# CityU-AIM-Group/HTD

Measured on AMD Instinct MI355X. Metric: images/sec (1333x800) HTD-R50 train step, higher is better.
Workload: dtype f32; 1 GPU; HTD ResNet-50 FPN fp32 train step fwd+bwd+SGD, batch 4/GPU @ 1333x800 (padded 1344x800), random-init weights, 2000 RPN proposals/img, 512 RoIs/img/stage; global_batch=4, parallelism=dp1, stage2_positives=158, proposals=random-init RPN (few positives: the regression branch is nearly idle)

## Files before the change

### htd_amd/csrc/conv_x3.hip

```cpp
#include <algorithm>
#include <mutex>
#include <type_traits>
#include <unordered_map>

#include <stdlib.h>

#include "common.h"

namespace {

using f32x16 = __attribute__((ext_vector_type(16))) float;
using bf16x8 = __attribute__((ext_vector_type(8))) __bf16;
using bf16x2 = __attribute__((ext_vector_type(2))) __bf16;
using f32x2 = __attribute__((ext_vector_type(2))) float;
using f32x4 = __attribute__((ext_vector_type(4))) float;

using f16x8 = __attribute__((ext_vector_type(8))) _Float16;
using f16x2 = __attribute__((ext_vector_type(2))) _Float16;

constexpr int XK = 16;
constexpr int NCH = 6;

struct H2Scale { float s, inv; };
__device__ __forceinline__ H2Scale h2_scale(const float *amax)
// ... 302 lines not shown
                *reinterpret_cast<float4 *>(p.y + o) = v;
                omax = absmax4(omax, v);
                if (p.yp != nullptr) emit_planes4(p.yp, p.yp_rows, m, n, v);
            } else {
                auto put = [&](int e, float t) {
                    if (n + e >= p.Co) return;
                    t += p.bias ? p.bias[n + e] : 0.f;
                    if (p.residual) t += p.residual[o + e];
                    if (p.relu) t = fmaxf(t, 0.f);
                    if (p.mask_src) t = p.mask_src[o + e] > 0.f ? t : 0.f;
                    p.y[o + e] = t;
                    omax = absmax4(omax, make_float4(t, 0.f, 0.f, 0.f));
                };
                put(0, v.x); put(1, v.y); put(2, v.z); put(3, v.w);
            }
        }
        if (i + 1 < TM) __syncthreads();
    }
    if (p.amax_out != nullptr && !part) block_absmax_out(omax, p.amax_out, le, oseen);
}

template <int WGM, int WGN, int TM, int TN, int KW, int NB, bool H2 = false>
constexpr int x3p_occupancy()
{
    constexpr int BM = WGM * TM * 32, BN = WGN * TN * 32;
    constexpr int NCHL = H2 ? 4 : NCH;
    constexpr int main_bytes = (2 * NCHL * Geo<BM, KW>::PITCH + NB * NCHL * BN) * 16;
    constexpr int epi_bytes = WGM * 32 * (BN + 4) * 4;
    constexpr int by_lds = 163840 / (main_bytes > epi_bytes ? main_bytes : epi_bytes);
    constexpr int by_regs = TM * TN >= 4 ? (H2 && HTD_X3H_OCC4 ? 4 : 3) : 4;
    return by_lds < by_regs ? by_lds : by_regs;
}

template <int WGM, int WGN, int TM, int TN, int KW, bool MF16, int NB, bool H2 = false>
__global__ __launch_bounds__(256, (x3p_occupancy<WGM, WGN, TM, TN, KW, NB, H2>())) void conv_x3p_kernel(X3Params p)
{
    static_assert(!(H2 && MF16), "H2: 32x32x16 form only");
    constexpr int NCHL = H2 ? 4 : NCH;
    constexpr int BM = WGM * TM * 32, BN = WGN * TN * 32;
    using G = Geo<BM, KW>;
    constexpr int PADX = (KW - 1) / 2;
    constexpr int A_VEC = NCHL * G::PITCH;
    constexpr int B_VEC = NCHL * BN;
    constexpr int MAIN_VEC = 2 * A_VEC + NB * B_VEC;
    constexpr int EPI_STRIDE = BN + 4, EPI_ROWS = WGM * 32;
    constexpr int EPI_VEC = EPI_ROWS * EPI_STRIDE / 4;
    constexpr int LDS_VEC = MAIN_VEC > EPI_VEC ? MAIN_VEC : EPI_VEC;
    __shared__ uint4 lds[LDS_VEC];
    uint4 *const lA = lds, *const lB = lds + 2 * A_VEC;
    const unsigned lds_a0 = (unsigned)(size_t)(__attribute__((address_space(3))) void *)lA;

    int bid = blockIdx.x, split = 0, sps = 0;
    bool part = false;
    const bool region_b = bid >= p.tiles_a * p.splits_a;
    if (region_b) {
        const int r = bid - p.tiles_a * p.splits_a;
        bid = p.tiles_a + r / p.splits_b;
        split = r % p.splits_b;
        part = p.splits_b > 1;
        sps = p.sps_b;
    } else if (p.splits_a > 1) {
        split = bid % p.splits_a;
        bid = bid / p.splits_a;
        part = true;
        sps = p.sps_a;
    } else {
        const int q = p.tiles_a / 8, r = p.tiles_a % 8, xcd = bid % 8, idx = bid / 8;
        bid = (xcd < r ? xcd * (q + 1) : r * (q + 1) + (xcd - r) * q) + idx;
    }
    const int tile_m = bid / p.nt, tile_n = bid % p.nt;
    const int64_t m0 = (int64_t)tile_m * BM;
    const int n0 = tile_n * BN;

    const int tid = threadIdx.x, lane = tid & 63, wave = tid >> 6;
    const int wm = wave / WGN, wn = wave % WGN;
    const int frow = lane & 31, fhalf = lane >> 5;
    const int PADY = (p.kh - 1) / 2;

    const int vcol = tid & 3, vrow = tid >> 2;
    const int a_g0 = (int)m0 + vrow - PADX;
    unsigned a_off[KW > 1 ? 1 : G::PASSES];
    bool a_in[KW > 1 ? 1 : G::PASSES];
    unsigned a_tm[KW > 1 ? 1 : G::PASSES];
    if constexpr (KW > 1) {
        a_off[0] = (unsigned)a_g0 * (unsigned)p.Ci + vcol * 4;
// ... 346 lines not shown
                    for (int i = 0; i < NP; ++i) store_pass(abuf ^ 1, i, (P ^ 1) * NP + i);
                } else {
                    store_pass(abuf ^ 1, kx, P ^ 1);
                }
            }
        }
        lds_barrier();
        bbuf = bbuf + 1 == NB ? 0 : bbuf + 1;
        if (++kx == KW) {
            kx = 0;
            ++s;
            abuf ^= 1;
            cs = cs1; ky = ky1;
            cs1 = cs2; ky1 = ky2;
            if (++ky2 == p.kh) { ky2 = 0; ++cs2; }
            n1shift = n2shift; n1koff = n2koff;
            n2shift = (ky2 - PADY) * p.Wx;
            n2koff = tap_koff(ky2, cs2);
        }
    };
    const int taps_total = (s_end - s_begin) * KW;
    int t = 0;
#pragma unroll 1
    for (; t + 1 < taps_total; t += 2) {
        tap(0, false);
        tap(1, false);
    }
    if (t < taps_total) tap(0, true);
    wait_vm<0>();
#pragma unroll
    for (int i = 0; i < 2 * NPT; ++i) landed(ra[i]);

    x3_epilogue<WGM, WGN, TM, TN, MF16>(p, acc, lds, m0, n0, part, region_b, split);
}

template <int WGM, int WGN, int TM, int TN, int NS>
constexpr int x3q_occupancy()
{
    constexpr int BM = WGM * TM * 32, BN = WGN * TN * 32;
    constexpr int main_bytes = NS * NCH * (BM + BN) * 16;
    constexpr int epi_bytes = WGM * 32 * (BN + 4) * 4;
    constexpr int by_lds = 163840 / (main_bytes > epi_bytes ? main_bytes : epi_bytes);
    constexpr int by_regs = TM * TN >= 4 ? 3 : 4;
    return by_lds < by_regs ? by_lds : by_regs;
}

template <int WGM, int WGN, int TM, int TN, bool MF16, int NS>
__global__ __launch_bounds__(256, (x3q_occupancy<WGM, WGN, TM, TN, NS>())) void conv_x3q_kernel(X3Params p)
{
    constexpr int BM = WGM * TM * 32, BN = WGN * TN * 32;
    constexpr int A_VEC = NCH * BM, B_VEC = NCH * BN;
    constexpr int MAIN_VEC = NS * (A_VEC + B_VEC);
    constexpr int EPI_VEC = WGM * 32 * (BN + 4) / 4;
    constexpr int LDS_VEC = MAIN_VEC > EPI_VEC ? MAIN_VEC : EPI_VEC;
    __shared__ uint4 lds[LDS_VEC];
    uint4 *const lA = lds, *const lB = lds + NS * A_VEC;
    const unsigned lds_a0 = (unsigned)(size_t)(__attribute__((address_space(3))) void *)lA;
    const unsigned lds_b0 = (unsigned)(size_t)(__attribute__((address_space(3))) void *)lB;

    int bid = blockIdx.x, split = 0, sps = 0;
    bool part = false;
    const bool region_b = bid >= p.tiles_a * p.splits_a;
    if (region_b) {
        const int r = bid - p.tiles_a * p.splits_a;
        bid = p.tiles_a + r / p.splits_b;
        split = r % p.splits_b;
// ... 737 lines not shown
        case 0: hipLaunchKernelGGL((conv_x3p_kernel<2, 2, 1, 1, 1, false, HTD_X3H_NB, true>), grid, dim3(256), 0, s, p); break;
        case 1: hipLaunchKernelGGL((conv_x3p_kernel<2, 2, 2, 2, 1, false, HTD_X3H_NB, true>), grid, dim3(256), 0, s, p); break;
        case 2: hipLaunchKernelGGL((conv_x3p_kernel<2, 2, 2, 1, 1, false, HTD_X3H_NB, true>), grid, dim3(256), 0, s, p); break;
        default: hipLaunchKernelGGL((conv_x3p_kernel<2, 2, 1, 2, 1, false, HTD_X3H_NB, true>), grid, dim3(256), 0, s, p); break;
        }
    } else if (p.xp != nullptr) {
        switch (cfg) {
        case 0: launch_tile_q<1, 1>(p, grid, s); break;
        case 1: launch_tile_q<2, 2>(p, grid, s); break;
        case 2: launch_tile_q<2, 1>(p, grid, s); break;
        default: launch_tile_q<1, 2>(p, grid, s); break;
        }
    } else {
        switch (cfg) {
        case 0: launch_tile<1, 1>(p, kw, grid, s); break;
        case 1: launch_tile<2, 2>(p, kw, grid, s); break;
        case 2: launch_tile<2, 1>(p, kw, grid, s); break;
        default: launch_tile<1, 2>(p, kw, grid, s); break;
        }
    }
    if (pl.partial_floats > 0) {
        const int64_t rows = (p.splits_a > 1 ? p.m_rem0 : 0) + (p.splits_b > 1 ? p.M - p.m_rem0 : 0);
        if ((p.Co & 3) == 0) {
            const unsigned rb = (unsigned)std::min<int64_t>(htd::ceil_div(rows * (p.Co >> 2), 256), p.amax_out ? 1024 : 4096);
            hipLaunchKernelGGL(conv_x3p_splitk_epilogue_vec_kernel, dim3(rb), dim3(256), 0, s, p);
        } else {
            const unsigned rb = (unsigned)std::min<int64_t>(htd::ceil_div(rows * p.Co, 256), p.amax_out ? 1024 : 4096);
            hipLaunchKernelGGL(conv_x3p_splitk_epilogue_kernel, dim3(rb), dim3(256), 0, s, p);
        }
    }
    return htd::check_launch("conv2d_x3p");
}

bool x3h_strided_ok(int Ci, int Co, int kh, int kw, int stride, int pad)
{
    static const bool on = !(getenv("HTD_X3H_STRIDED") && atoi(getenv("HTD_X3H_STRIDED")) == 0);
    return on && Ci % XK == 0 && Co >= 33 && kh == 3 && kw == 3 && stride == 2 && pad == 1;
}

bool x3p_shape_ok(int Ci, int Co, int kh, int kw, int stride, int pad, int dil)
{
    if (Ci % XK != 0 || Co < 33 || dil != 1 || kh != kw) return false;
    if (kh == 1) return pad == 0 && stride >= 1;
    return kh == 3 && stride == 1 && pad == 1;
}

}

extern "C" int htd_conv2d_x3p_supported(int Ci, int Co, int kh, int kw, int stride, int pad, int dil)
{
    return (!x3p_off() && htd::conv_math() == 1 && x3p_shape_ok(Ci, Co, kh, kw, stride, pad, dil)) ? 1 : 0;
}

int g_conv_h2 = getenv("HTD_CONV_H2") ? atoi(getenv("HTD_CONV_H2")) : 1;
extern "C" int htd_conv2d_set_h2(int on)
{
    const int prev = g_conv_h2;
    if (on == 0 || on == 1) g_conv_h2 = on;
    return prev;
}
extern "C" int htd_conv2d_x3h_supported(int Ci, int Co, int kh, int kw, int stride, int pad, int dil)
{
    return (g_conv_h2 == 1 && htd_conv2d_x3p_supported(Ci, Co, kh, kw, stride, pad, dil)) ? 1 : 0;
}
extern "C" int htd_conv2d_x3h_strided_supported(int Ci, int Co, int kh, int kw, int stride, int pad, int dil)
{
// ... 221 lines not shown
        p.res_H = res_h; p.res_W = res_w;
        p.res_sh = (float)res_h / (float)p.Ho; p.res_sw = (float)res_w / (float)p.Wo;
    }
    if (taps) {
        p.kh = p.ntl = kh * kw;
        for (int t = 0; t < p.ntl; ++t) { p.tl_dy[t] = t / kw - pad; p.tl_dx[t] = t % kw - pad; p.tl_w[t] = t; }
        return launch_x3p(p, 1, (hipStream_t)stream, workspace);
    }
    return launch_x3p(p, kw, (hipStream_t)stream, workspace);
}

extern "C" int htd_conv2d_bwd_data_x3h(const float *gy, const float *amax, const void *wplanesT, const float *mask_src,
                                       const float *accum, float *gx, void *gxplanes, float *amax_out, int B, int H, int W,
                                       int Ci, int Co, int kh, int kw, int pad, void *workspace, void *stream)
{
    HTD_REQUIRE(!gxplanes || Ci % XK == 0, "conv2d_bwd_data_x3h: output planes need Ci %% 16 == 0 (Ci=%d)", Ci);
    HTD_REQUIRE(gy && amax && wplanesT && gx && B > 0 && H > 0 && W > 0, "conv2d_bwd_data_x3h: bad arguments");
    HTD_REQUIRE(x3p_shape_ok(Co, Ci, kh, kw, 1, pad, 1), "conv2d_bwd_data_x3h: unsupported layer Ci=%d Co=%d k=%dx%d p=%d", Ci, Co, kh,
                kw, pad);
    X3Params p{};
    p.x = gy; p.wp = (const uint4 *)wplanesT; p.residual = accum; p.mask_src = mask_src; p.y = gx;
    p.Hx = H; p.Wx = W; p.Ho = H; p.Wo = W;
    p.Ci = Co; p.Co = Ci; p.Cop = planes_np(Ci); p.kh = kh; p.stride = 1;
    p.M = (int64_t)B * H * W;
    p.ncs = Co / XK;
    p.amax = amax;
    p.wscale = reinterpret_cast<const float *>(p.wp + planes_vec(kh * kw, Co, p.Cop));
    p.yp = (uint4 *)gxplanes; p.yp_rows = act_rows(p.M);
    p.amax_out = amax_out;
    HTD_REQUIRE((int64_t)B * H * W * Co < (1ll << 31), "conv2d_bwd_data_x3h: operand too large");
    return launch_x3p(p, kw, (hipStream_t)stream, workspace);
}

namespace {
struct StridedClass { int ntaps; int dy[9], dx[9], w[9]; int Ho, Wo; };
int strided_classes(int H, int W, int kh, int kw, int stride, int pad, StridedClass *cls)
{
    int n = 0;
    for (int c = 0; c < stride * stride; ++c) {
        const int ph = c / stride, pw = c % stride;
        StridedClass &q = cls[c];
        q.ntaps = 0;
        q.Ho = ph < H ? (H - ph + stride - 1) / stride : 0;
        q.Wo = pw < W ? (W - pw + stride - 1) / stride : 0;
        if (q.Ho == 0 || q.Wo == 0) continue;
        for (int ky = 0; ky < kh; ++ky) {
            const int ry = ph + pad - ky;
            if (((ry % stride) + stride) % stride != 0) continue;
            for (int kx = 0; kx < kw; ++kx) {
                const int rx = pw + pad - kx;
                if (((rx % stride) + stride) % stride != 0) continue;
                q.dy[q.ntaps] = ry >= 0 ? ry / stride : -((-ry) / stride);
                q.dx[q.ntaps] = rx >= 0 ? rx / stride : -((-rx) / stride);
                q.w[q.ntaps] = (kh - 1 - ky) * kw + (kw - 1 - kx);
                ++q.ntaps;
            }
        }
        n += q.ntaps > 0;
    }
    return n;
}
bool x3h_strided_dgrad_ok(int Ci, int Co, int kh, int kw, int stride, int pad)
{
    static const bool on = !(getenv("HTD_X3H_STRIDED") && atoi(getenv("HTD_X3H_STRIDED")) == 0);
    return on && Co % XK == 0 && Ci >= 33 && stride == 2 && ((kh == 3 && kw == 3 && pad == 1) || (kh == 1 && kw == 1 && pad == 0));
}
}

extern "C" int htd_conv2d_bwd_data_x3h_strided_supported(int Ci, int Co, int kh, int kw, int stride, int pad, int dil)
{
    return (g_conv_h2 == 1 && !x3p_off() && htd::conv_math() == 1 && dil == 1 && x3h_strided_dgrad_ok(Ci, Co, kh, kw, stride, pad)) ? 1 : 0;
}

extern "C" int64_t htd_conv2d_bwd_data_x3h_strided_workspace_bytes(int B, int H, int W, int Ci, int Co, int kh, int kw, int stride, int pad)
{
    if (!x3h_strided_dgrad_ok(Ci, Co, kh, kw, stride, pad) || B <= 0 || H <= 0 || W <= 0) return 0;
    StridedClass cls[4];
    strided_classes(H, W, kh, kw, stride, pad, cls);
    int64_t need = 0;
    for (int c = 0; c < stride * stride; ++c)
        if (cls[c].ntaps > 0)
            need = std::max(need, htd_conv2d_x3p_workspace_bytes((int64_t)B * cls[c].Ho * cls[c].Wo, Ci, Co, cls[c].ntaps, 1));
    return need;
}

extern "C" int htd_conv2d_bwd_data_x3h_strided(const float *gy, const float *amax, const void *wplanesT, const float *mask_src,
                                               float *gx, float *amax_out, int B, int H, int W, int Ci, int Co, int kh, int kw,
                                               int stride, int pad, void *workspace, void *stream)
{
    HTD_REQUIRE(gy && amax && wplanesT && gx && B > 0 && H > 0 && W > 0, "conv2d_bwd_data_x3h_strided: bad arguments");
    HTD_REQUIRE(x3h_strided_dgrad_ok(Ci, Co, kh, kw, stride, pad), "conv2d_bwd_data_x3h_strided: unsupported layer Ci=%d Co=%d k=%dx%d s=%d p=%d",
                Ci, Co, kh, kw, stride, pad);
    const int Ho = (H + 2 * pad - kh) / stride + 1, Wo = (W + 2 * pad - kw) / stride + 1;
    HTD_REQUIRE(Ho > 0 && Wo > 0 && (int64_t)B * Ho * Wo * Co < (1ll << 31) && (int64_t)B * H * W * Ci < (1ll << 40),
                "conv2d_bwd_data_x3h_strided: bad sizes");
    StridedClass cls[4];
    const int live = strided_classes(H, W, kh, kw, stride, pad, cls);
    if (live < stride * stride) {
        if (hipMemsetAsync(gx, 0, (size_t)B * H * W * Ci * 4, (hipStream_t)stream) != hipSuccess) {
            htd::set_error("conv2d_bwd_data_x3h_strided: memset failed");
            return HTD_ERR_LAUNCH;
        }
    }
    X3Params p{};
    p.x = gy; p.wp = (const uint4 *)wplanesT; p.mask_src = mask_src; p.y = gx;
    p.Hx = Ho; p.Wx = Wo;
    p.Ci = Co; p.Co = Ci; p.Cop = planes_np(Ci); p.stride = 1;
    p.ncs = Co / XK;
    p.amax = amax;
    p.wscale = reinterpret_cast<const float *>(p.wp + planes_vec(kh * kw, Co, p.Cop));
    p.amax_out = amax_out;
    p.o_step = stride; p.oH = H; p.oW = W;
    for (int c = 0; c < stride * stride; ++c) {
        const StridedClass &q = cls[c];
        if (q.ntaps == 0) continue;
        X3Params r = p;
        r.Ho = q.Ho; r.Wo = q.Wo;
        r.M = (int64_t)B * q.Ho * q.Wo;
        r.kh = r.ntl = q.ntaps;
        for (int t = 0; t < q.ntaps; ++t) { r.tl_dy[t] = q.dy[t]; r.tl_dx[t] = q.dx[t]; r.tl_w[t] = q.w[t]; }
        r.o_h0 = c / stride; r.o_w0 = c % stride;
        const int st = launch_x3p(r, 1, (hipStream_t)stream, workspace);
        if (st) return st;
    }
    return HTD_OK;
}
```

### htd_amd/dense.py

```python
import os

import torch
from torch.autograd import Function
from torch.autograd.function import once_differentiable
from torch.multiprocessing.reductions import StorageWeakRef as _StorageWeakRef

from . import capi
from .mmcv_ops import chain_outputs

CL = torch.channels_last
_P = capi.ptr
_S = capi.current_stream_ptr


def _out_hw(H, W, kh, kw, stride, pad, dil):
    return ((H + 2 * pad - (dil * (kh - 1) + 1)) // stride + 1, (W + 2 * pad - (dil * (kw - 1) + 1)) // stride + 1)


def _need_gpu(t, name):
    if not t.is_cuda:
        raise NotImplementedError(f'{name}: only GPU tensors are supported (libhtd_amd.so has no CPU path)')


def _splitk_ws(M, Co, Cred, kh, kw, device):
    nbytes = capi.lib().htd_conv2d_workspace_bytes(M, Co, Cred, kh, kw)
    return torch.empty(nbytes // 4, device=device, dtype=torch.float32) if nbytes > 0 else None


_GRAD_SINK = {}


def register_grad_sinks(params, views, used):
# ... 739 lines not shown
    else:
        capi.call('htd_conv2d_bwd_weight', _P(x), _P(g), _P(gw), _P(gb), B, H, W, Ci, Co, kh, kw, stride, padding,
                  dilation, _P(ws), _S(), work=work)
    return gw, gb, sink_w and sink_b


def _wgrad_raw(x, g, weight, stride, padding, dilation, bias=None, overlap=True):
    amax = _wgrad_amax(x, g, weight, stride, padding, dilation)
    if not overlap or not OVERLAP_WGRAD or (capi.profiling() and not _OVERLAP_IN_PROFILE):
        if OVERLAP_WGRAD and _SIDE and SINK_ACCUMULATE and grad_sink_again(weight) is not None:
            torch.cuda.current_stream().wait_stream(side_stream(g.device))
        return _wgrad_launch(x, g, weight, stride, padding, dilation, bias, amax)[:2]
    main, side = torch.cuda.current_stream(), side_stream(g.device)
    side.wait_stream(main)
    x.record_stream(side)
    g.record_stream(side)
    with torch.cuda.stream(side):
        gw, gb, sinks = _wgrad_launch(x, g, weight, stride, padding, dilation, bias, amax)
    if not sinks and not side_consumed(weight):
        if gw is not None:
            gw.record_stream(main)
        if gb is not None:
            gb.record_stream(main)
        main.wait_stream(side)
    return gw, gb


def _dgrad_joined(galias, g, weight, x_shape, stride, padding, dilation):
    fuse = galias is not None and stride == 1 and galias.dtype == g.dtype and tuple(galias.shape) == tuple(x_shape)
    gx = _dgrad_raw(g, weight, x_shape, stride, padding, dilation, accum=galias.contiguous(memory_format=CL) if fuse else None)
    return gx if (galias is None or fuse) else gx + galias


class Conv2dFunction(Function):
    @staticmethod
    def forward(ctx, x, weight, bias, residual, stride, padding, dilation, relu, res_up=False, chain=False):
        _need_gpu(x, 'conv2d')
        src = x
        x = x.contiguous(memory_format=CL)
        weight = weight.contiguous(memory_format=CL)
        res = residual.contiguous(memory_format=CL) if residual is not None else None
        b = bias.contiguous() if bias is not None else None
        y = _fwd_raw(x, weight, b, res, stride, padding, dilation, relu, res_up)
        ctx.save_for_backward(x, weight, y if relu else None)
        ctx.cfg = (stride, padding, dilation, bool(relu), bias is not None, residual is not None)
        ctx.res_up = tuple(res.shape) if (res_up and res is not None) else None
        ctx.bias_ref = b
        return chain_outputs(ctx, y, (src, ), chain)

    @staticmethod
    @once_differentiable
    def backward(ctx, g, galias=None):
        x, weight, y = ctx.saved_tensors
        stride, padding, dilation, relu, has_bias, has_res = ctx.cfg
        if g is None:
            return (galias, ) + (None, ) * 9
        g = g.contiguous(memory_format=CL)
        need_x, need_w, need_b, need_r = ctx.needs_input_grad[:4]
        gb = gw = None
        want_b = has_bias and need_b
        if relu:
            if want_b and not need_w:
                g, gb = _colsum_raw(g, y, ctx.bias_ref)
            else:
                g = _mask_raw(g, y)
        elif want_b and not need_w:
# ... 25 lines not shown
        b1 = b1.contiguous() if b1 is not None else None
        b2 = b2.contiguous() if b2 is not None else None
        h = _fwd_raw(x, w1, b1, None, 1, padding, 1, True)
        y = _fwd_raw(h, w2, b2, None, 1, 0, 1, False)
        ctx.save_for_backward(x, w1, w2, h)
        ctx.cfg = (int(padding), b1, b2)
        return chain_outputs(ctx, y, (src, ), chain)

    @staticmethod
    @once_differentiable
    def backward(ctx, gy, galias=None):
        x, w1, w2, h = ctx.saved_tensors
        padding, b1, b2 = ctx.cfg
        if gy is None:
            return (galias, ) + (None, ) * 6
        need_x, need_w1, need_b1, need_w2, need_b2 = ctx.needs_input_grad[:5]
        gy = gy.contiguous(memory_format=CL)
        gw1 = gb1 = gw2 = gb2 = None
        if need_w2:
            gw2, gb2 = _wgrad_raw(h, gy, w2, 1, 0, 1, b2 if (need_b2 and b2 is not None) else None)
        elif need_b2 and b2 is not None:
            gb2 = _colsum_raw(gy, None, b2)[1]
        gh = _dgrad_raw(gy, w2, h.shape, 1, 0, 1, mask_src=h)
        if need_w1:
            gw1, gb1 = _wgrad_raw(x, gh, w1, 1, padding, 1, b1 if (need_b1 and b1 is not None) else None)
        elif need_b1 and b1 is not None:
            gb1 = _colsum_raw(gh, None, b1)[1]
        gx = _dgrad_joined(galias, gh, w1, x.shape, 1, padding, 1) if need_x else galias
        return gx, gw1, gb1, gw2, gb2, None, None


def conv_relu_head(x, w1, b1, w2, b2, padding=1, chain=False):
    return ConvReluHeadFunction.apply(x, w1, b1, w2, b2, int(padding), bool(chain))



def _gconv_pack(weight, groups, transpose):
    C, cg, kh, kw = weight.shape
    n = capi.lib().htd_gconv2d_packed_floats(C, groups, kh, kw)
    if n <= 0:
        raise ValueError(f'grouped conv2d: {C} channels in {groups} groups is unsupported')
    wp = torch.empty(n, device=weight.device, dtype=weight.dtype)
    capi.call('htd_gconv2d_pack_weights', _P(weight), _P(wp), C, groups, kh, kw, int(transpose), _S())
    return wp


def _gconv_fwd_raw(x, wp, bias, geom, relu, cols_shape=None):
    C, groups, kh, kw, stride, padding, dilation = geom
    B, H, W = cols_shape if cols_shape is not None else (x.size(0), x.size(2), x.size(3))
    Ho, Wo = _out_hw(H, W, kh, kw, stride, padding, dilation)
    y = torch.empty((B, C, Ho, Wo), device=x.device, dtype=x.dtype, memory_format=CL)
    capi.call('htd_gconv2d_fwd', _P(x), _P(wp), _P(bias), _P(y), B, H, W, C, groups, kh, kw, stride, padding, dilation,
              int(bool(relu)), int(cols_shape is not None), _S(),
              work=('flop', 2.0 * B * Ho * Wo * C * kh * kw * (C // groups), 4.0 * (x.numel() + y.numel())))
    return y


def _gconv_dgrad_raw(g, wpT, geom, x_shape, cols=False):
    C, groups, kh, kw, stride, padding, dilation = geom
    B, _, H, W = x_shape
    M = g.size(0) * g.size(2) * g.size(3)
    gx = torch.empty((M, kh * kw, C), device=g.device, dtype=g.dtype) if cols else \
        torch.empty((B, C, H, W), device=g.device, dtype=g.dtype, memory_format=CL)
    capi.call('htd_gconv2d_bwd_data', _P(g), _P(wpT), _P(gx), B, H, W, C, groups, kh, kw, stride, padding, dilation,
              int(cols), _S(), work=('flop', 2.0 * M * C * kh * kw * (C // groups), 4.0 * (g.numel() + gx.numel())))
    return gx
# ... 565 lines not shown
```

### htd_amd/detector/rpn_head.py

```python
import torch

from ..core import multi_apply
from ..core.bbox import delta2bbox_clip_device
from ..core.misc import arange_cached, const_tensor
from .. import mmcv_ops as M
from ..mmcv_ops import nms_sorted_mask
from ..registry import HEADS
from .anchor_heads import AnchorHead
from .bricks import Conv2d, normal_init


class _RPNLossFunction(torch.autograd.Function):

    @staticmethod
    def forward(ctx, cls, reg, anchors, gts, assigned, pos, neg, means, stds, beta, pos_weight):
        from .. import capi
        from ..core.bbox import _f4
        B, A = assigned.shape
        K = gts.size(1)
        cls, reg = cls.float().contiguous(), reg.float().contiguous()
        anchors, gts = anchors.float().contiguous(), gts.float().contiguous()
        assigned = assigned.contiguous()
        pos8, neg8 = pos.to(torch.uint8).contiguous(), neg.to(torch.uint8).contiguous()
        partial = torch.empty(capi.lib().htd_rpn_loss_partial_rows(), 2, device=cls.device, dtype=torch.float32)
# ... 92 lines not shown
        super().__init__(1, in_channels, **kwargs)
        assert self.use_sigmoid_cls and not self.reg_decoded_bbox, 'HTD configs use a sigmoid RPN with delta targets'

    def _init_layers(self):
        self.rpn_conv = Conv2d(self.in_channels, self.feat_channels, 3, padding=1)
        self.rpn_cls = Conv2d(self.feat_channels, self.num_anchors * self.cls_out_channels, 1)
        self.rpn_reg = Conv2d(self.feat_channels, self.num_anchors * 4, 1)

    def init_weights(self):
        normal_init(self.rpn_conv, std=0.01)
        normal_init(self.rpn_cls, std=0.01)
        normal_init(self.rpn_reg, std=0.01)

    def forward_single(self, x):
        x = self.rpn_conv(x, relu=True)
        if x.dtype != torch.float32:
            x = x.float()
        return self.rpn_cls(x), self.rpn_reg(x)

    def forward(self, feats):
        if not feats[0].is_cuda:
            return multi_apply(self.forward_single, feats)
        nc, nr = self.rpn_cls.out_channels, self.rpn_reg.out_channels
        pad = -(nc + nr) % 8
        w = torch.cat([self.rpn_cls.weight, self.rpn_reg.weight] +
                      ([self.rpn_cls.weight.new_zeros(pad, *self.rpn_cls.weight.shape[1:])] if pad else []))
        b = torch.cat([self.rpn_cls.bias, self.rpn_reg.bias] + ([self.rpn_cls.bias.new_zeros(pad)] if pad else []))
        cls, reg, merged = [], [], []
        taps = isinstance(feats, M.PyramidTaps)
        from .. import dense
        if torch.is_grad_enabled() and w.requires_grad:
            dense.temp_grad_sink(w)
            dense.temp_grad_sink(b)
        for i in range(len(feats)):
            x = feats[i]
            if x.dtype == torch.float32 and x.size(1) % 8 == 0:
                conv = (self.rpn_conv.weight, self.rpn_conv.bias, w, b, self.rpn_conv.padding[0])
                y = feats.tap(lambda f: dense.conv_relu_head(f, *conv, True), i)[0] if taps else dense.conv_relu_head(x, *conv)
            else:
                h = self.rpn_conv(x, relu=True)
                if h.dtype != torch.float32:
                    h = h.float()
                y = self.rpn_cls(h, weight=w, bias=b)
            merged.append(y)
        if RPN_FLAT_HEADS and self.cls_out_channels == 1 and nr == 4 * nc and all(y.dtype == torch.float32 for y in merged):
            cls_all, reg_all = _RPNGatherHeads.apply(nc, *merged)
            cls, reg, off = LevelList(), LevelList(), 0
            B = cls_all.size(0)
            for y in merged:
                hh, ww = y.size(2), y.size(3)
                n = hh * ww * nc
                cls.append(cls_all[:, off:off + n].view(B, hh, ww, nc).permute(0, 3, 1, 2))
                reg.append(reg_all[:, off:off + n].reshape(B, hh, ww, nr).permute(0, 3, 1, 2))
                off += n
            cls.flat, reg.flat = cls_all, reg_all
            return cls, reg
        for y in merged:
            c, r = _SplitHeads.apply(y, nc, nr)
            cls.append(c)
            reg.append(r)
        return cls, reg

    def simple_test_rpn(self, x, img_metas):
        return self.get_bboxes(*self(x), img_metas)

    def aug_test_rpn(self, feats, img_metas):
        from ..core.post_processing import merge_aug_proposals
        samples_per_gpu = len(img_metas[0])
        aug_proposals = [[] for _ in range(samples_per_gpu)]
        for x, img_meta in zip(feats, img_metas):
# ... 201 lines not shown
```

### include/htd_amd.h

```cpp
#ifndef HTD_AMD_H
#define HTD_AMD_H

#include <stdint.h>

#ifdef __cplusplus
extern "C" {
#endif

#define HTD_OK 0
#define HTD_ERR_ARG 1
#define HTD_ERR_LAUNCH 2

const char *htd_last_error(void);
#define HTD_ABI_VERSION 8
int htd_abi_version(void);

int htd_roi_align_fwd(const float *feat, const float *rois, const int64_t *roi_level, int level,
                      float *out, int64_t n, int B, int C, int H, int W, int ph, int pw, float spatial_scale,
                      int sampling_ratio, int aligned, void *stream);
int htd_roi_align_bwd(const float *grad_out, const float *rois, const int64_t *roi_level, int level,
                      float *grad_feat, int64_t n, int B, int C, int H, int W, int ph, int pw,
                      float spatial_scale, int sampling_ratio, int aligned, void *stream);
int htd_roi_align_levels_fwd(const float *const *feats, const int *H, const int *W, const float *scales, int L,
                             const float *rois, const int64_t *roi_level, float *out, int64_t n, int B, int C, int ph, int pw,
// ... 108 lines not shown
int htd_conv2d_x3p_plan_query(int cfg, int64_t M, int Co, int Ci, int kh, int kw, int64_t *out);
int64_t htd_conv2d_x3_planes_bytes(int Co, int kh, int kw, int Ci, int transposed);
int htd_conv2d_x3_planes(const float *w, void *planes, int Co, int kh, int kw, int Ci, int transposed, void *stream);
int htd_conv2d_x3_planes_many(const void *desc, int n, int64_t total_blocks, void *stream);
int64_t htd_conv2d_x3p_workspace_bytes(int64_t M, int Co, int Ci, int kh, int kw);
int htd_conv2d_fwd_x3p(const float *x, const void *wplanes, const float *bias, const float *residual, int res_h,
                       int res_w, float *y, int B, int H, int W, int Ci, int Co, int kh, int kw, int stride, int pad,
                       int relu, void *workspace, void *stream);
int htd_conv2d_bwd_data_x3p(const float *gy, const void *wplanesT, const float *mask_src, const float *accum,
                            float *gx, int B, int H, int W, int Ci, int Co, int kh, int kw, int pad, void *workspace,
                            void *stream);
int64_t htd_act_planes_rows(int64_t M);
int64_t htd_act_planes_bytes(int64_t M, int C);
int htd_act_planes(const float *x, void *planes, int64_t M, int C, void *stream);
int htd_conv2d_fwd_x3q(const float *x, const void *xplanes, const void *wplanes, const float *bias, const float *residual,
                       int res_h, int res_w, float *y, void *yplanes, float *amax_out, int B, int H, int W, int Ci, int Co, int kh, int kw,
                       int stride, int pad, int relu, void *workspace, void *stream);
int htd_conv2d_bwd_data_x3q(const float *gy, const void *gyplanes, const void *wplanesT, const float *mask_src,
                            const float *accum, float *gx, void *gxplanes, float *amax_out, int B, int H, int W, int Ci, int Co, int kh, int kw,
                            int pad, void *workspace, void *stream);

int htd_conv2d_set_h2(int on);
int htd_conv2d_bwd_weight_h2_supported(int B, int H, int W, int Ci, int Co, int kh, int kw, int stride, int pad, int dil);
int htd_conv2d_bwd_weight_h2(const float *x, const float *gy, const float *amax_x, const float *amax_g, float *gw,
                             float *gbias, int B, int H, int W, int Ci, int Co, int kh, int kw, int stride, int pad,
                             int dil, int accumulate, void *workspace, void *stream);
int htd_conv2d_x3h_supported(int Ci, int Co, int kh, int kw, int stride, int pad, int dil);
int htd_conv2d_x3h_strided_supported(int Ci, int Co, int kh, int kw, int stride, int pad, int dil);
int htd_conv2d_bwd_data_x3h_strided_supported(int Ci, int Co, int kh, int kw, int stride, int pad, int dil);
int64_t htd_conv2d_bwd_data_x3h_strided_workspace_bytes(int B, int H, int W, int Ci, int Co, int kh, int kw, int stride, int pad);
int htd_conv2d_bwd_data_x3h_strided(const float *gy, const float *amax, const void *wplanesT, const float *mask_src, float *gx,
                                    float *amax_out, int B, int H, int W, int Ci, int Co, int kh, int kw, int stride, int pad,
                                    void *workspace, void *stream);
int htd_absmax(const float *x, int64_t n, float *amax, void *stream);
int htd_conv2d_x3h_planes(const float *w, void *planes, int Co, int kh, int kw, int Ci, int transposed, void *stream);
int htd_conv2d_x3h_planes_many(const void *desc, int n, int64_t total_blocks, int64_t total_rows, void *stream);
int htd_conv2d_fwd_x3h(const float *x, const float *amax, const void *wplanes, const float *bias, const float *residual,
                       int res_h, int res_w, float *y, void *yplanes, float *amax_out, int B, int H, int W, int Ci,
                       int Co, int kh, int kw, int stride, int pad, int relu, void *workspace, void *stream);
int htd_conv2d_bwd_data_x3h(const float *gy, const float *amax, const void *wplanesT, const float *mask_src,
                            const float *accum, float *gx, void *gxplanes, float *amax_out, int B, int H, int W,
                            int Ci, int Co, int kh, int kw, int pad, void *workspace, void *stream);

int64_t htd_deform_columns_bytes(int B, int H, int W, int C, int kh, int kw, int stride, int pad, int dil);
int htd_deform_im2col(const float *x, const float *offset, const float *mask, float *columns, int B,
                      int H, int W, int C, int kh, int kw, int stride, int pad, int dil,
                      int deform_groups, void *stream);
int htd_deform_col2im(const float *x, const float *offset, const float *mask, const float *gcolumns,
                      float *gx, float *goffset, float *gmask, int B, int H, int W, int C, int kh,
                      int kw, int stride, int pad, int dil, int deform_groups, void *stream);
int htd_deform_im2col_bf16(const void *x, const float *offset, const float *mask, void *columns, int B, int H, int W,
                           int C, int kh, int kw, int stride, int pad, int dil, int deform_groups, void *stream);
int htd_deform_col2im_bf16(const void *x, const float *offset, const float *mask, const void *gcolumns, float *gx,
                           float *goffset, float *gmask, int B, int H, int W, int C, int kh, int kw, int stride, int pad,
                           int dil, int deform_groups, void *stream);

int htd_global_avg_pool_fwd(const float *x, float *out, int64_t B, int P, int C, void *stream);
int htd_global_avg_pool_bwd(const float *g, float *gx, int64_t B, int P, int C, void *stream);
int htd_global_avg_pool_bwd_acc(const float *g, float *gx, int64_t B, int P, int C, void *stream);

int htd_group_norm_relu_fwd(const float *x, const float *gamma, const float *beta, float *y,
                            float *mean, float *rstd, int64_t n, int P, int C, int G, float eps,
                            int relu, void *stream);
int htd_group_norm_relu_bwd(const float *x, const float *y, const float *gamma, const float *mean,
                            const float *rstd, const float *gy, float *gx, float *ggamma,
                            float *gbeta, int64_t n, int P, int C, int G, int relu, void *stream);
// ... 295 lines not shown
```

Before: 122.5 images/sec.

## Batch multi-level RPN and strided dgrad convs into one grouped table kernel

Adds a grouped-GEMM style conv kernel that takes a table of up to eight same-weight-shape problems and maps each block to its problem by tile offset. The RPN head's 3x3 conv across FPN levels (forward and data-gradient) and the strided data-gradient sub-convolutions now launch as one kernel when the total tile count is large enough. The aim is to cut per-level launch overhead and fill the GPU with the small-level tiles. The trade-off is that one tile config is chosen for the largest problem and split-K is dropped for all members.

```diff
diff --git a/htd_amd/csrc/conv_x3.hip b/htd_amd/csrc/conv_x3.hip
--- a/htd_amd/csrc/conv_x3.hip
+++ b/htd_amd/csrc/conv_x3.hip
@@ -358,8 +358,8 @@
     return by_lds < by_regs ? by_lds : by_regs;
 }
 
-template <int WGM, int WGN, int TM, int TN, int KW, bool MF16, int NB, bool H2 = false>
-__global__ __launch_bounds__(256, (x3p_occupancy<WGM, WGN, TM, TN, KW, NB, H2>())) void conv_x3p_kernel(X3Params p)
+template <int WGM, int WGN, int TM, int TN, int KW, bool MF16, int NB, bool H2>
+__device__ __forceinline__ void conv_x3p_tile(const X3Params &p, int bid)
 {
     static_assert(!(H2 && MF16), "H2: 32x32x16 form only");
     constexpr int NCHL = H2 ? 4 : NCH;
@@ -376,7 +376,7 @@
     uint4 *const lA = lds, *const lB = lds + 2 * A_VEC;
     const unsigned lds_a0 = (unsigned)(size_t)(__attribute__((address_space(3))) void *)lA;
 
-    int bid = blockIdx.x, split = 0, sps = 0;
+    int split = 0, sps = 0;
     bool part = false;
     const bool region_b = bid >= p.tiles_a * p.splits_a;
     if (region_b) {
@@ -789,6 +789,30 @@
     for (int i = 0; i < 2 * NPT; ++i) landed(ra[i]);
 
     x3_epilogue<WGM, WGN, TM, TN, MF16>(p, acc, lds, m0, n0, part, region_b, split);
+}
+
+template <int WGM, int WGN, int TM, int TN, int KW, bool MF16, int NB, bool H2 = false>
+__global__ __launch_bounds__(256, (x3p_occupancy<WGM, WGN, TM, TN, KW, NB, H2>())) void conv_x3p_kernel(X3Params p)
+{
+    conv_x3p_tile<WGM, WGN, TM, TN, KW, MF16, NB, H2>(p, blockIdx.x);
+}
+
+constexpr int X3T_MAX = 8;
+struct X3Table {
+    X3Params prob[X3T_MAX];
+    int tile_end[X3T_MAX];
+};
+static_assert(sizeof(X3Table) <= 4096, "the problem table must fit the kernel argument segment");
+
+template <int WGM, int WGN, int TM, int TN, int KW, int NB>
+__global__ __launch_bounds__(256, (x3p_occupancy<WGM, WGN, TM, TN, KW, NB, true>())) void conv_x3t_kernel(X3Table t)
+{
+    const int b = blockIdx.x;
+    int i = 0;
+#pragma unroll
+    for (int k = 0; k + 1 < X3T_MAX; ++k) i += b >= t.tile_end[k] ? 1 : 0;
+    i = __builtin_amdgcn_readfirstlane(i);
+    conv_x3p_tile<WGM, WGN, TM, TN, KW, false, NB, true>(t.prob[i], b - (i ? t.tile_end[i - 1] : 0));
 }
 
 template <int WGM, int WGN, int TM, int TN, int NS>
@@ -1592,6 +1616,76 @@
     return htd::check_launch("conv2d_x3p");
 }
 
+int g_x3_table = getenv("HTD_X3_TABLE") ? std::min(std::max(atoi(getenv("HTD_X3_TABLE")), 0), 2) : 1;
+
+int table_cfg_of(const X3Params *probs, int n, int kw)
+{
+    int big = 0;
+    for (int i = 1; i < n; ++i)
+        if (probs[i].M > probs[big].M) big = i;
+    const X3Params &q = probs[big];
+    const int epi = (q.residual ? 1 : 0) | (q.mask_src ? 2 : 0) | 4;
+    return choose_cfg(q.M, q.Co, q.Ci, q.kh * kw + (q.ntl > 0 ? 100 : 0), epi);
+}
+bool table_planned(const X3Params *probs, int n, int kw)
+{
+    if (!g_x3_table || n < 2 || n > X3T_MAX) return false;
+    if (g_x3_table == 2) return true;
+    const int cfg = table_cfg_of(probs, n, kw);
+    int64_t tiles = 0;
+    for (int i = 0; i < n; ++i) tiles += htd::ceil_div(probs[i].M, kXCfg[cfg].bm) * htd::ceil_div(probs[i].Co, kXCfg[cfg].bn);
+    return tiles > 256 * kXOcc[cfg];
+}
+
+int launch_x3_table(const X3Params *probs, int n, int kw, hipStream_t s)
+{
+    HTD_REQUIRE(n >= 1 && n <= X3T_MAX, "conv2d_x3 table: %d problems (1 .. %d)", n, X3T_MAX);
+    const int cfg = table_cfg_of(probs, n, kw);
+    int order[X3T_MAX];
+    for (int i = 0; i < n; ++i) order[i] = i;
+    std::stable_sort(order, order + n, [&](int a, int b) {
+        const int ka = probs[a].ncs * probs[a].kh, kb = probs[b].ncs * probs[b].kh;
+        return ka != kb ? ka > kb : probs[a].M > probs[b].M;
+    });
+    X3Table t{};
+    int64_t tiles = 0;
+    for (int k = 0; k < X3T_MAX; ++k) {
+        if (k >= n) { t.tile_end[k] = 0x7fffffff; continue; }
+        X3Params &p = t.prob[k];
+        p = probs[order[k]];
+        HTD_REQUIRE(p.amax && p.wscale && p.M > 0 && p.xp == nullptr && p.yp == nullptr && p.res_H == 0,
+                    "conv2d_x3 table: problem %d is not a plain H2 problem", order[k]);
+        HTD_REQUIRE(p.Ci == probs[0].Ci && p.Co == probs[0].Co && (p.ntl > 0) == (probs[0].ntl > 0) && (p.ntl > 0 || p.kh == probs[0].kh) &&
+                        p.stride == probs[0].stride,
+                    "conv2d_x3 table: problem %d differs from problem 0 in Ci / Co / filter form", order[k]);
+        p.mt = (int)htd::ceil_div(p.M, kXCfg[cfg].bm);
+        p.nt = (int)htd::ceil_div(p.Co, kXCfg[cfg].bn);
+        p.tiles_a = p.mt * p.nt; p.splits_a = 1; p.sps_a = p.ncs * p.kh; p.splits_b = 1; p.sps_b = p.sps_a;
+        p.m_rem0 = p.M;
+        p.partial = nullptr;
+        tiles += p.tiles_a;
+        HTD_REQUIRE(tiles < (1ll << 31) - 1, "conv2d_x3 table: bad grid");
+        t.tile_end[k] = (int)tiles;
+    }
+    const dim3 grid((unsigned)tiles);
+    if (kw == 3) {
+        switch (cfg) {
+        case 0: hipLaunchKernelGGL((conv_x3t_kernel<2, 2, 1, 1, 3, HTD_X3H_NB>), grid, dim3(256), 0, s, t); break;
+        case 1: hipLaunchKernelGGL((conv_x3t_kernel<2, 2, 2, 2, 3, HTD_X3H_NB>), grid, dim3(256), 0, s, t); break;
+        case 2: hipLaunchKernelGGL((conv_x3t_kernel<2, 2, 2, 1, 3, HTD_X3H_NB>), grid, dim3(256), 0, s, t); break;
+        default: hipLaunchKernelGGL((conv_x3t_kernel<2, 2, 1, 2, 3, HTD_X3H_NB>), grid, dim3(256), 0, s, t); break;
+        }
+    } else {
+        switch (cfg) {
+        case 0: hipLaunchKernelGGL((conv_x3t_kernel<2, 2, 1, 1, 1, HTD_X3H_NB>), grid, dim3(256), 0, s, t); break;
+        case 1: hipLaunchKernelGGL((conv_x3t_kernel<2, 2, 2, 2, 1, HTD_X3H_NB>), grid, dim3(256), 0, s, t); break;
+        case 2: hipLaunchKernelGGL((conv_x3t_kernel<2, 2, 2, 1, 1, HTD_X3H_NB>), grid, dim3(256), 0, s, t); break;
+        default: hipLaunchKernelGGL((conv_x3t_kernel<2, 2, 1, 2, 1, HTD_X3H_NB>), grid, dim3(256), 0, s, t); break;
+        }
+    }
+    return htd::check_launch("conv2d_x3 table");
+}
+
 bool x3h_strided_ok(int Ci, int Co, int kh, int kw, int stride, int pad)
 {
     static const bool on = !(getenv("HTD_X3H_STRIDED") && atoi(getenv("HTD_X3H_STRIDED")) == 0);
@@ -1879,6 +1973,83 @@
     return launch_x3p(p, kw, (hipStream_t)stream, workspace);
 }
 
+extern "C" int htd_conv2d_x3_table_set(int on)
+{
+    const int prev = g_x3_table;
+    if (on >= 0 && on <= 2) g_x3_table = on;
+    return prev;
+}
+
+namespace {
+int table_problems(const htd_x3h_problem *d, int n, bool dgrad, int B, int Ci, int Co, int kh, int kw, int pad, int relu, X3Params *out)
+{
+    const char *who = dgrad ? "conv2d_bwd_data_x3h_table" : "conv2d_fwd_x3h_table";
+    HTD_REQUIRE(d && n >= 1 && n <= X3T_MAX && B > 0, "%s: %d problems (1 .. %d)", who, n, X3T_MAX);
+    HTD_REQUIRE(dgrad ? x3p_shape_ok(Co, Ci, kh, kw, 1, pad, 1) : x3p_shape_ok(Ci, Co, kh, kw, 1, pad, 1),
+                "%s: unsupported layer Ci=%d Co=%d k=%dx%d p=%d", who, Ci, Co, kh, kw, pad);
+    const int K = dgrad ? Co : Ci, N = dgrad ? Ci : Co;
+    for (int i = 0; i < n; ++i) {
+        const htd_x3h_problem &q = d[i];
+        HTD_REQUIRE(q.x && q.amax && q.wplanes && q.y && q.H > 0 && q.W > 0, "%s: problem %d: null operand or empty map", who, i);
+        HTD_REQUIRE(dgrad ? q.bias == nullptr : q.mask_src == nullptr, "%s: problem %d: %s", who, i,
+                    dgrad ? "a data gradient takes no bias" : "a forward takes no mask");
+        HTD_REQUIRE((int64_t)B * q.H * q.W * K < (1ll << 31) && (int64_t)B * q.H * q.W * N < (1ll << 40), "%s: problem %d: operand too large",
+                    who, i);
+        X3Params p{};
+        p.x = q.x; p.wp = (const uint4 *)q.wplanes; p.bias = q.bias; p.residual = q.residual; p.mask_src = q.mask_src; p.y = q.y;
+        p.Hx = p.Ho = (int)q.H; p.Wx = p.Wo = (int)q.W;
+        p.Ci = K; p.Co = N; p.Cop = planes_np(N); p.kh = kh; p.stride = 1; p.relu = dgrad ? 0 : relu;
+        p.M = (int64_t)B * q.H * q.W;
+        p.ncs = K / XK;
+        p.amax = q.amax;
+        p.wscale = reinterpret_cast<const float *>(p.wp + planes_vec(kh * kw, K, p.Cop));
+        p.amax_out = q.amax_out;
+        out[i] = p;
+    }
+    return HTD_OK;
+}
+int table_or_each(const X3Params *probs, int n, int kw, int mode, void *workspace, hipStream_t s)
+{
+    if (mode < 0) mode = table_planned(probs, n, kw) ? 1 : 0;
+    if (mode == 1) return launch_x3_table(probs, n, kw, s);
+    for (int i = 0; i < n; ++i) {
+        const int st = launch_x3p(probs[i], kw, s, workspace);
+        if (st) return st;
+    }
+    return HTD_OK;
+}
+}
+
+extern "C" int htd_conv2d_x3h_table_planned(const int64_t *H, const int64_t *W, int n, int B, int Ci, int Co, int kh, int kw, int pad,
+                                            int dgrad)
+{
+    if (!H || !W || n < 1 || n > X3T_MAX || g_conv_h2 != 1 || !htd_conv2d_x3p_supported(dgrad ? Co : Ci, dgrad ? Ci : Co, kh, kw, 1, pad, 1))
+        return 0;
+    X3Params probs[X3T_MAX] = {};
+    for (int i = 0; i < n; ++i) {
+        if (H[i] <= 0 || W[i] <= 0 || B <= 0) return 0;
+        probs[i].M = (int64_t)B * H[i] * W[i];
+        probs[i].Ci = dgrad ? Co : Ci; probs[i].Co = dgrad ? Ci : Co; probs[i].kh = kh;
+    }
+    return table_planned(probs, n, kw) ? 1 : 0;
+}
+
+extern "C" int htd_conv2d_fwd_x3h_table(const htd_x3h_problem *probs, int n, int B, int Ci, int Co, int kh, int kw, int pad, int relu,
+                                        int mode, void *workspace, void *stream)
+{
+    X3Params p[X3T_MAX];
+    const int st = table_problems(probs, n, false, B, Ci, Co, kh, kw, pad, relu, p);
+    return st ? st : table_or_each(p, n, kw, mode, workspace, (hipStream_t)stream);
+}
+
+extern "C" int htd_conv2d_bwd_data_x3h_table(const htd_x3h_problem *probs, int n, int B, int Ci, int Co, int kh, int kw, int pad,
+                                             int mode, void *workspace, void *stream)
+{
+    X3Params p[X3T_MAX];
+    const int st = table_problems(probs, n, true, B, Ci, Co, kh, kw, pad, 0, p);
+    return st ? st : table_or_each(p, n, kw, mode, workspace, (hipStream_t)stream);
+}
+
 namespace {
 struct StridedClass { int ntaps; int dy[9], dx[9], w[9]; int Ho, Wo; };
 int strided_classes(int H, int W, int kh, int kw, int stride, int pad, StridedClass *cls)
@@ -1931,9 +2102,9 @@
     return need;
 }
 
-extern "C" int htd_conv2d_bwd_data_x3h_strided(const float *gy, const float *amax, const void *wplanesT, const float *mask_src,
-                                               float *gx, float *amax_out, int B, int H, int W, int Ci, int Co, int kh, int kw,
-                                               int stride, int pad, void *workspace, void *stream)
+extern "C" int htd_conv2d_bwd_data_x3h_strided_mode(const float *gy, const float *amax, const void *wplanesT, const float *mask_src,
+                                                    float *gx, float *amax_out, int B, int H, int W, int Ci, int Co, int kh, int kw,
+                                                    int stride, int pad, void *workspace, void *stream, int mode)
 {
     HTD_REQUIRE(gy && amax && wplanesT && gx && B > 0 && H > 0 && W > 0, "conv2d_bwd_data_x3h_strided: bad arguments");
     HTD_REQUIRE(x3h_strided_dgrad_ok(Ci, Co, kh, kw, stride, pad), "conv2d_bwd_data_x3h_strided: unsupported layer Ci=%d Co=%d k=%dx%d s=%d p=%d",
@@ -1958,17 +2129,26 @@
     p.wscale = reinterpret_cast<const float *>(p.wp + planes_vec(kh * kw, Co, p.Cop));
     p.amax_out = amax_out;
     p.o_step = stride; p.oH = H; p.oW = W;
+    X3Params probs[4];
+    int n = 0;
     for (int c = 0; c < stride * stride; ++c) {
         const StridedClass &q = cls[c];
         if (q.ntaps == 0) continue;
-        X3Params r = p;
+        X3Params &r = probs[n++];
+        r = p;
         r.Ho = q.Ho; r.Wo = q.Wo;
         r.M = (int64_t)B * q.Ho * q.Wo;
         r.kh = r.ntl = q.ntaps;
         for (int t = 0; t < q.ntaps; ++t) { r.tl_dy[t] = q.dy[t]; r.tl_dx[t] = q.dx[t]; r.tl_w[t] = q.w[t]; }
         r.o_h0 = c / stride; r.o_w0 = c % stride;
-        const int st = launch_x3p(r, 1, (hipStream_t)stream, workspace);
-        if (st) return st;
-    }
-    return HTD_OK;
-}
+    }
+    return n ? table_or_each(probs, n, 1, mode, workspace, (hipStream_t)stream) : HTD_OK;
+}
+
+extern "C" int htd_conv2d_bwd_data_x3h_strided(const float *gy, const float *amax, const void *wplanesT, const float *mask_src,
+                                               float *gx, float *amax_out, int B, int H, int W, int Ci, int Co, int kh, int kw,
+                                               int stride, int pad, void *workspace, void *stream)
+{
+    return htd_conv2d_bwd_data_x3h_strided_mode(gy, amax, wplanesT, mask_src, gx, amax_out, B, H, W, Ci, Co, kh, kw, stride, pad,
+                                                workspace, stream, -1);
+}
diff --git a/htd_amd/dense.py b/htd_amd/dense.py
--- a/htd_amd/dense.py
+++ b/htd_amd/dense.py
@@ -1,3 +1,4 @@
+import ctypes
 import os
 
 import torch
@@ -803,6 +804,89 @@
     return gx if (galias is None or fuse) else gx + galias
 
 
+X3_TABLE_MAX = 8
+
+
+def _table_members(ts, weights, dgrad, padding):
+    Co, Ci, kh, kw = weights[0].shape
+    cred, cout = (Co, Ci) if dgrad else (Ci, Co)
+    if not (2 <= len(ts) <= X3_TABLE_MAX) or kh != kw or any(tuple(w.shape) != tuple(weights[0].shape) for w in weights) or \
+            any(t.dtype != torch.float32 or t.size(0) != ts[0].size(0) or t.numel() == 0 for t in ts) or \
+            not _x3h_ok(cred, cout, kh, kw, 1, padding, 1, ts[0].dtype):
+        return {}
+    ams = {}
+    for i, t in enumerate(ts):
+        am = carried_amax(t)
+        if am is None:
+            _h2_trace('dgrad' if dgrad else 'fwd', t, weights[i])
+            if kh * kw * cout >= H2_ABSMAX_MIN_WORK and t.numel() >= H2_ABSMAX_MIN_ELEMS:
+                am = absmax(t)
+        if am is not None:
+            ams[i] = am
+    if len(ams) < 2:
+        return {}
+    hs = (ctypes.c_int64 * len(ams))(*[ts[i].size(2) for i in ams])
+    wss = (ctypes.c_int64 * len(ams))(*[ts[i].size(3) for i in ams])
+    planned = capi.lib().htd_conv2d_x3h_table_planned(ctypes.cast(hs, ctypes.c_void_p), ctypes.cast(wss, ctypes.c_void_p), len(ams),
+                                                      ts[0].size(0), Ci, Co, kh, kw, padding, int(dgrad))
+    return ams if planned else {}
+
+
+def _table_call(name, rows, ints, key, work):
+    desc = (ctypes.c_int64 * (10 * len(rows)))(*[(v.data_ptr() if torch.is_tensor(v) else (v or 0)) for r in rows for v in r])
+    capi.call(name, ctypes.cast(desc, ctypes.c_void_p), len(rows), *ints, 1, None, _S(), key=key, work=work)
+
+
+def _fwd_table_raw(xs, weights, biases, residuals, padding, relu):
+    n = len(xs)
+    Co, Ci, kh, kw = weights[0].shape
+    ams = _table_members(xs, weights, False, padding)
+    ys = [None if i in ams else _fwd_raw(xs[i], weights[i], biases[i], residuals[i], 1, padding, 1, relu) for i in range(n)]
+    if ams:
+        B = xs[0].size(0)
+        rows, slots, flops, nbytes = [], {}, 0.0, 0.0
+        planes = [x3_planes(weights[i], False, True) for i in ams]
+        for (i, am), pl in zip(ams.items(), planes):
+            x, H, W = xs[i], xs[i].size(2), xs[i].size(3)
+            ys[i] = torch.empty((B, Co, H, W), device=x.device, dtype=x.dtype, memory_format=CL)
+            slots[i] = _amax_slot(x.device)
+            rows.append((x, am, pl, biases[i], residuals[i], None, ys[i], slots[i], H, W))
+            flops += 2.0 * B * H * W * Co * kh * kw * Ci
+            nbytes += 4.0 * (x.numel() + weights[i].numel() + ys[i].numel() * (1 + (residuals[i] is not None)))
+        _table_call('htd_conv2d_fwd_x3h_table', rows, (B, Ci, Co, kh, kw, padding, int(bool(relu))),
+                    'htd_conv2d_fwd_x3h', ('flop', flops, nbytes))
+        for i, am in ams.items():
+            tag_amax(ys[i], slots[i])
+            _h2_guard(am, slots[i])
+    return ys
+
+
+def _dgrad_table_raw(gs, weights, x_shapes, padding, mask_srcs, accums):
+    n = len(gs)
+    Co, Ci, kh, kw = weights[0].shape
+    ams = _table_members(gs, weights, True, padding)
+    gxs = [None if i in ams else _dgrad_raw(gs[i], weights[i], x_shapes[i], 1, padding, 1, mask_src=mask_srcs[i], accum=accums[i])
+           for i in range(n)]
+    if ams:
+        B = gs[0].size(0)
+        rows, slots, flops, nbytes = [], {}, 0.0, 0.0
+        planes = [x3_planes(weights[i], True, True) for i in ams]
+        for (i, am), pl in zip(ams.items(), planes):
+            g, H, W = gs[i], x_shapes[i][2], x_shapes[i][3]
+            gxs[i] = torch.empty((B, Ci, H, W), device=g.device, dtype=g.dtype, memory_format=CL)
+            slots[i] = _amax_slot(g.device)
+            rows.append((g, am, pl, None, accums[i], mask_srcs[i], gxs[i], slots[i], H, W))
+            flops += 2.0 * B * H * W * Co * kh * kw * Ci
+            nbytes += 4.0 * (g.numel() + weights[i].numel() +
+                             gxs[i].numel() * (1 + (mask_srcs[i] is not None) + (accums[i] is not None)))
+        _table_call('htd_conv2d_bwd_data_x3h_table', rows, (B, Ci, Co, kh, kw, padding),
+                    'htd_conv2d_bwd_data_x3h', ('flop', flops, nbytes))
+        for i, am in ams.items():
+            tag_amax(gxs[i], slots[i])
+            _h2_guard(am, slots[i])
+    return gxs
+
+
 class Conv2dFunction(Function):
     @staticmethod
     def forward(ctx, x, weight, bias, residual, stride, padding, dilation, relu, res_up=False, chain=False):
@@ -894,6 +978,75 @@
 
 def conv_relu_head(x, w1, b1, w2, b2, padding=1, chain=False):
     return ConvReluHeadFunction.apply(x, w1, b1, w2, b2, int(padding), bool(chain))
+
+
+def _add_grads(a, b):
+    return b if a is None else (a if b is None else a + b)
+
+
+class ConvReluHeadLevelsFunction(Function):
+
+    @staticmethod
+    def forward(ctx, w1, b1, w2, b2, padding, chain, *xs):
+        n = len(xs)
+        for x in xs:
+            _need_gpu(x, 'conv_relu_head_levels')
+        srcs = xs
+        xs = [x.contiguous(memory_format=CL) for x in xs]
+        w1, w2 = w1.contiguous(memory_format=CL), w2.contiguous(memory_format=CL)
+        b1 = b1.contiguous() if b1 is not None else None
+        b2 = b2.contiguous() if b2 is not None else None
+        hs = _fwd_table_raw(xs, [w1] * n, [b1] * n, [None] * n, padding, True)
+        ys = tuple(_fwd_raw(h, w2, b2, None, 1, 0, 1, False) for h in hs)
+        ctx.save_for_backward(w1, w2, *xs, *hs)
+        ctx.cfg = (int(padding), b1, b2, n)
+        return chain_outputs(ctx, ys, srcs, chain)
+
+    @staticmethod
+    @once_differentiable
+    def backward(ctx, *grads):
+        padding, b1, b2, n = ctx.cfg
+        w1, w2 = ctx.saved_tensors[:2]
+        xs, hs = ctx.saved_tensors[2:2 + n], ctx.saved_tensors[2 + n:2 + 2 * n]
+        gys = grads[:n]
+        galias = list(grads[n:]) if len(grads) > n else [None] * n
+        need_w1, need_b1, need_w2, need_b2 = ctx.needs_input_grad[:4]
+        need_x = ctx.needs_input_grad[6:]
+        gw1 = gb1 = gw2 = gb2 = None
+        gxs, live, ghs = list(galias), [], []
+        for i in reversed(range(n)):
+            if gys[i] is None:
+                continue
+            gy, h = gys[i].contiguous(memory_format=CL), hs[i]
+            if need_w2:
+                a, b = _wgrad_raw(h, gy, w2, 1, 0, 1, b2 if (need_b2 and b2 is not None) else None)
+                gw2, gb2 = _add_grads(gw2, a), _add_grads(gb2, b)
+            elif need_b2 and b2 is not None:
+                gb2 = _add_grads(gb2, _colsum_raw(gy, None, b2)[1])
+            gh = _dgrad_raw(gy, w2, h.shape, 1, 0, 1, mask_src=h)
+            if need_w1:
+                a, b = _wgrad_raw(xs[i], gh, w1, 1, padding, 1, b1 if (need_b1 and b1 is not None) else None)
+                gw1, gb1 = _add_grads(gw1, a), _add_grads(gb1, b)
+            elif need_b1 and b1 is not None:
+                gb1 = _add_grads(gb1, _colsum_raw(gh, None, b1)[1])
+            if need_x[i]:
+                live.append(i)
+                ghs.append(gh)
+        if live:
+            fuse = [galias[i] is not None and galias[i].dtype == ghs[k].dtype and tuple(galias[i].shape) == tuple(xs[i].shape)
+                    for k, i in enumerate(live)]
+            acc = [galias[i].contiguous(memory_format=CL) if f else None for i, f in zip(live, fuse)]
+            if len(live) > 1:
+                out = _dgrad_table_raw(ghs, [w1] * len(live), [xs[i].shape for i in live], padding, [None] * len(live), acc)
+            else:
+                out = [_dgrad_raw(ghs[0], w1, xs[live[0]].shape, 1, padding, 1, accum=acc[0])]
+            for k, i in enumerate(live):
+                gxs[i] = out[k] if (galias[i] is None or fuse[k]) else out[k] + galias[i]
+        return (gw1, gb1, gw2, gb2, None, None, *gxs)
+
+
+def conv_relu_head_levels(xs, w1, b1, w2, b2, padding=1, chain=False):
+    return ConvReluHeadLevelsFunction.apply(w1, b1, w2, b2, int(padding), bool(chain), *xs)
 
 
 
diff --git a/htd_amd/detector/rpn_head.py b/htd_amd/detector/rpn_head.py
--- a/htd_amd/detector/rpn_head.py
+++ b/htd_amd/detector/rpn_head.py
@@ -148,10 +148,16 @@
         if torch.is_grad_enabled() and w.requires_grad:
             dense.temp_grad_sink(w)
             dense.temp_grad_sink(b)
-        for i in range(len(feats)):
+        n = len(feats)
+        conv = (self.rpn_conv.weight, self.rpn_conv.bias, w, b, self.rpn_conv.padding[0])
+        if 2 <= n <= dense.X3_TABLE_MAX and all(feats[i].dtype == torch.float32 and feats[i].size(1) % 8 == 0 for i in range(n)):
+            if taps:
+                merged = list(feats.tap(lambda *fs: dense.conv_relu_head_levels(fs, *conv, True), 0, n))
+            else:
+                merged = list(dense.conv_relu_head_levels([feats[i] for i in range(n)], *conv))
+        for i in range(n if not merged else 0):
             x = feats[i]
             if x.dtype == torch.float32 and x.size(1) % 8 == 0:
-                conv = (self.rpn_conv.weight, self.rpn_conv.bias, w, b, self.rpn_conv.padding[0])
                 y = feats.tap(lambda f: dense.conv_relu_head(f, *conv, True), i)[0] if taps else dense.conv_relu_head(x, *conv)
             else:
                 h = self.rpn_conv(x, relu=True)
diff --git a/include/htd_amd.h b/include/htd_amd.h
--- a/include/htd_amd.h
+++ b/include/htd_amd.h
@@ -164,6 +164,26 @@
 int htd_conv2d_bwd_data_x3h_strided(const float *gy, const float *amax, const void *wplanesT, const float *mask_src, float *gx,
                                     float *amax_out, int B, int H, int W, int Ci, int Co, int kh, int kw, int stride, int pad,
                                     void *workspace, void *stream);
+int htd_conv2d_bwd_data_x3h_strided_mode(const float *gy, const float *amax, const void *wplanesT, const float *mask_src, float *gx,
+                                         float *amax_out, int B, int H, int W, int Ci, int Co, int kh, int kw, int stride, int pad,
+                                         void *workspace, void *stream, int mode);
+typedef struct htd_x3h_problem {
+    const float *x;
+    const float *amax;
+    const void *wplanes;
+    const float *bias;
+    const float *residual;
+    const float *mask_src;
+    float *y;
+    float *amax_out;
+    int64_t H, W;
+} htd_x3h_problem;
+int htd_conv2d_x3_table_set(int on);
+int htd_conv2d_x3h_table_planned(const int64_t *H, const int64_t *W, int n, int B, int Ci, int Co, int kh, int kw, int pad, int dgrad);
+int htd_conv2d_fwd_x3h_table(const htd_x3h_problem *probs, int n, int B, int Ci, int Co, int kh, int kw, int pad, int relu, int mode,
+                             void *workspace, void *stream);
+int htd_conv2d_bwd_data_x3h_table(const htd_x3h_problem *probs, int n, int B, int Ci, int Co, int kh, int kw, int pad, int mode,
+                                  void *workspace, void *stream);
 int htd_absmax(const float *x, int64_t n, float *amax, void *stream);
 int htd_conv2d_x3h_planes(const float *w, void *planes, int Co, int kh, int kw, int Ci, int transposed, void *stream);
 int htd_conv2d_x3h_planes_many(const void *desc, int n, int64_t total_blocks, int64_t total_rows, void *stream);
```

New measurement: 123.9 images/sec (median of 5 runs). +1.2%, better.
